# davidesantangelo/krep

Measured on AMD Instinct MI355X. Metric: GB/s scanned (literal scan, match offsets produced), haystack resident in HBM, higher is better.
Workload: dtype u8; 1 GPU; literal8: 8-byte case-sensitive literal 'Sherlock', ~1e-4 matches/byte, offsets tracked; 32 GiB per GPU (BASELINE.json configs[1]); pattern=Sherlock, bytes_per_gpu=34359738368, matches=3436005, parallelism=contiguous shards x1, start-offset ownership, 1 RCCL all-reduce of counts

## Files before the change

include/krep_gpu_debug.h:

```cpp
#ifndef KREP_GPU_DEBUG_H
#define KREP_GPU_DEBUG_H
#include "krep_gpu.h"
#ifdef __cplusplus
extern "C" {
#endif

uint64_t krep_gpu_debug_replay_host(int krep_ref_algo, const void *text, size_t n, const void *pattern, uint32_t m,
                                    int whole_word, size_t cur, int open_line);
void krep_gpu_debug_force_rounds(int rounds);
void krep_gpu_debug_force_stage_cap(int records);
void krep_gpu_debug_force_single_grid(int blocks);
uint64_t krep_gpu_debug_single_failovers(void);
uint64_t krep_gpu_debug_single_launches(void);
uint64_t krep_gpu_debug_tiny_launches(void);
uint64_t krep_gpu_debug_tiny_dense_launches(void);
void krep_gpu_debug_inject_failure(int kind);
void krep_gpu_debug_chain_fixups(uint64_t *rescans, uint64_t *replays);
void krep_gpu_debug_fold_carry(const krep_gpu_seq_carry_t *in, const krep_gpu_seq_carry_t *piece, krep_gpu_seq_carry_t *out);
uint64_t krep_gpu_debug_anchored_launches(void);
uint64_t krep_gpu_debug_literal_dma_launches(void);
int krep_gpu_debug_literal_dma_state(const krep_gpu_plan_t *plan, int *looked, int *barred, double *pass_rate);
uint64_t krep_gpu_debug_runs_launches(void);
int krep_gpu_debug_split_state(const krep_gpu_plan_t *plan);
int krep_gpu_debug_anchor_info(const krep_gpu_plan_t *plan, int *state, uint32_t *moved, double *rate_end_grams, double *rate_anchors);
int krep_gpu_debug_anchor_measured(const krep_gpu_plan_t *plan, double *measured, int *resamples);

#ifdef __cplusplus
}
#endif
#endif
```

krep_amd/csrc/kg_ac.hip:

```cpp
#include <hip/hip_runtime.h>

#include <algorithm>
#include <atomic>
#include <cstdlib>
#include <cstring>
#include <unordered_map>
#include <vector>

#include "../../include/krep_gpu.h"
#include "kg_ac_common.h"
#include "kg_ac_tables.h"
#include "kg_internal.h"

namespace kg {

#ifndef KG_AC_LINES_ROLL_CELLS
#define KG_AC_LINES_ROLL_CELLS 4
#endif
template <bool CI, bool LINES, bool SHORT, int STRIDE, int ANCH = 0, bool WW = false>
__global__ __launch_bounds__(kAcBlock) void ac_scan_kernel(const AcArgs a)
{
    static_assert(!WW || (STRIDE == 2 && !SHORT), "the -w filter of the depth masks: pair filter, no short patterns");
    static_assert(!ANCH || (STRIDE == 2 && !LINES && !SHORT), "anchored scan: pair filter, records / counts only");
    extern __shared__ __attribute__((aligned(16))) u32 s_mem[];
// ... 1177 lines not shown
    const u32 waves = r.tiny ? (u32)kTinyWaves : (u32)kAcWaves;
    a.upt = (u32)std::min<u64>(kAcUnitsPerTicketMax, std::max<u64>(1, a.num_tiles / ((u64)c.num_cu * waves * 4)));
    if (const char *e = getenv("KREP_GPU_AC_UPT"))
    {
        const int v = atoi(e);
        if (v >= 1 && v <= (int)kAcUnitsPerTicketMax)
            a.upt = (u32)v;
    }
    if (c.time_it) HIPCHK(hipEventRecord(c.ev0, c.st));
    const bool dbg_sync = getenv("KREP_GPU_SYNC_DEBUG") != nullptr;
    auto dbg = [&](const char *what) -> int {
        if (!dbg_sync)
            return 0;
        const hipError_t e = hipStreamSynchronize(c.st);
        return e == hipSuccess ? 0 : fail("ac_scan: %s faulted: %s (tiny=%d stride=%u units=%llu stage_cap=%u lines=%d list=%d own=[%llu,%llu) end=[%llu,%llu) n=%llu)", what,
                                          hipGetErrorString(e), (int)r.tiny, a.stride, (unsigned long long)n_units, a.stage_cap, (int)c.lines, (int)r.lines_on_list,
                                          (unsigned long long)a.own_lo, (unsigned long long)a.own_hi, (unsigned long long)a.end_lo,
                                          (unsigned long long)a.end_hi, (unsigned long long)c.text_len);
    };
    HIPCHK(hipMemsetAsync(c.d_ctr, 0, sizeof(Counters), c.st));
    HIPCHK(ac_staged_launch(c, r, a));
    if (dbg("scan kernel")) return 2;
    if (chain && post_order(*c.post, n_units, a.stage_cap, 0, a.anchor + c.global_base, kAcUnitBytes, c.lines, (uint64_t *)c.d_pos, r.want, c.d_ctr,
                            c.num_cu, c.st))
        return 2;
    if (dbg("post-pass")) return 2;
    if (r.lines_on_list && r.want && tail_launch_line_gaps(c.d_text, c.text_len, c.global_base, (const uint64_t *)c.d_pos, &c.d_ctr->total,
                                                           &c.d_ctr->overflow_units, r.want, &c.d_ctr->lines, c.st))
        return 2;
    if (dbg("line-gap kernel")) return 2;
    if (c.time_it) HIPCHK(hipEventRecord(c.ev1, c.st));
    HIPCHK(hipMemcpyAsync(c.h_ctr, c.d_ctr, sizeof(Counters), hipMemcpyDeviceToHost, c.st));
    HIPCHK(hipStreamSynchronize(c.st));
    return 0;
}
static void ac_learn(const AcScan &c, const AcRun &r)
{
    AcTables *t = c.t;
    const AcArgs &a = r.a;
    const Counters &h = *c.h_ctr;
    const size_t own_lo = c.own_lo, own_hi = r.own_hi;
    const u64 n_units = a.num_tiles;
    if (!r.tiny && !c.lines && a.stride == 2 && own_hi > own_lo)
    {
        const double tested = 0.5 * (double)(own_hi - own_lo);
        t->anch_measured = (double)h.candidates / tested;
        const double est = t->anch_state == 2 ? t->anch_rate : t->anch_rate0;
        if (t->anch_state != 0 && t->anch_resamples < kAnchResamples && c.text_len >= (1u << 20) && own_hi - own_lo >= (1u << 19) &&
            t->anch_measured > 0.008 && t->anch_measured > 2.0 * est + 0.002 && !getenv("KREP_GPU_AC_ANCHOR") && !getenv("KREP_GPU_AC_NO_RESAMPLE"))
        {
            if (getenv("KREP_GPU_DEBUG"))
                fprintf(stderr, "krep-gpu: anchors: measured %.3f %% candidates per tested position against %.3f %% estimated (%s): the next scan decides again\n",
                        100.0 * t->anch_measured, 100.0 * est, t->anch_state == 2 ? "anchored" : "end grams");
            t->anch_state = 0;
            ++t->anch_resamples;
        }
    }
    if (!r.want || r.fsc)
        return;
    if (r.tiny && h.overflow_units * 2 > n_units && h.total > n_units * 256)
        t->stage_cap = 0;
    else if (t->stage_cap && h.overflow_units * 64 > n_units)
        t->stage_cap = 64;
    else if (!t->stage_cap && h.total < n_units * 32)
        t->stage_cap = 64;
    if (r.tiny)
// ... 47 lines not shown
```

krep_amd/csrc/kg_internal.h:

```cpp
#pragma once
#include <hip/hip_runtime.h>

#include <atomic>
#include <cstring>
#include <initializer_list>
#include <mutex>
#include <vector>

#include "../../include/krep_gpu.h"
#include "../../include/krep_gpu_debug.h"
#include "kg_common.h"

namespace kg {

int fail(const char *fmt, ...);
const char *device_unusable(int device);
bool inject(int kind);
#define HIPCHK(x)                                                                                 \
    do                                                                                            \
    {                                                                                             \
        hipError_t e_ = (x);                                                                      \
        if (e_ != hipSuccess)                                                                     \
            return kg::fail("%s failed: %s (%s:%d)", #x, hipGetErrorString(e_), __FILE__, __LINE__); \
    } while (0)
// ... 29 lines not shown
    (void)hipGetDevice(&dev);
    const bool known = dev >= 0 && dev < 64;
    if (known && granted[dev].load(std::memory_order_acquire))
        return hipSuccess;
    const hipError_t e = hipFuncSetAttribute(reinterpret_cast<const void *>(Kernel), hipFuncAttributeMaxDynamicSharedMemorySize, bytes);
    if (e == hipSuccess && known)
        granted[dev].store(true, std::memory_order_release);
    return e;
}

hipError_t launch_literal(const LitArgs &a, uint32_t num_cu, hipStream_t st);
int runs_count_greedy(const uint8_t *d_text, uint64_t text_len, uint64_t lo, uint64_t hi, uint32_t m, uint8_t byte, bool ci, int num_cu,
                      unsigned long long *d_slots, unsigned long long *h_slots, hipStream_t st, uint64_t *total, uint64_t *end_p1);
bool literal_dma_eligible(const LitArgs &a);
hipError_t launch_literal_dma(const LitArgs &a, uint32_t num_cu, hipStream_t st);
hipError_t launch_dma_byte_look(const uint8_t *text, uint64_t lo, uint32_t n_cells, uint32_t prefilter, bool ci, unsigned long long *out, hipStream_t st);
extern std::atomic<uint64_t> g_runs_launches;
extern std::atomic<uint64_t> g_lit_dma_launches;

struct PostScratch;
constexpr int kFusedShapeMax = 5;
double single_fused_max_density(int shape);
int single_fused_shape_for(double density, double margin, int start);
bool single_fused_reopens(uint64_t total, uint64_t span);
constexpr int kFusedGaveUp = 1;
int single_fused_run(const LitArgs &a, uint64_t n_units, uint64_t span, PostScratch &post, Counters *d_ctr, Counters *h_ctr,
                     uint32_t num_cu, int *shape, hipEvent_t ev_end, hipStream_t st, bool count_launch);

struct PostScratch
{
    unsigned long long *d_unitinfo = nullptr;
    unsigned long long *d_offsets = nullptr;
    unsigned long long *d_blk = nullptr;
    uint64_t units_cap = 0;
    unsigned long long *d_stage = nullptr;
    uint64_t stage_cap_words = 0;
    uint64_t *d_occ = nullptr;
    uint64_t occ_cap = 0;
    uint8_t *d_keep = nullptr;
    unsigned long long *d_gblk = nullptr;
    unsigned long long *d_surv = nullptr;
    uint64_t keep_cap = 0;
    unsigned long long *d_tk = nullptr;
    uint64_t tk_cap = 0;
};
void post_free(PostScratch &s);
int post_reserve(PostScratch &s, uint64_t n_units, uint64_t stage_words);
int post_order(PostScratch &s, uint64_t n_units, uint32_t stage_cap, uint32_t fixed_len, uint64_t origin, uint64_t unit_bytes,
               bool want_lines, uint64_t *d_pos, uint64_t pos_cap, Counters *d_ctr, int num_cu, hipStream_t st);
int post_offsets_pass(PostScratch &s, uint64_t n_units, bool want_lines, Counters *d_ctr, hipStream_t st);
int post_gather_pass(PostScratch &s, uint64_t n_units, uint32_t stage_cap, uint32_t fixed_len, uint64_t origin,
                     uint64_t unit_bytes, uint64_t *d_pos, uint64_t pos_cap, int num_cu, hipStream_t st);
constexpr uint32_t kWalkGreedy = 0;
constexpr uint32_t kWalkShortO = 1;
constexpr uint32_t kWalkShortOLines = 2;
struct WalkSpec
{
    uint32_t mode, m;
    bool ww, lines, ci;
    uint8_t b1, b2;
};
int post_walk(PostScratch &s, const uint8_t *d_text, uint64_t text_len, uint64_t global_base, const WalkSpec &ws,
              uint64_t n_occ, uint64_t *d_pos, uint64_t want, Counters *d_ctr, Counters *h_ctr, hipStream_t st,
              uint64_t *total, uint64_t *nlines, uint64_t *resume);

constexpr uint32_t kNlWalkSse42 = 0, kNlWalkKmp = 1;
int post_nlwalk(PostScratch &s, const uint8_t *d_text, uint64_t text_len, uint32_t mode, uint32_t m, uint32_t k0, bool ww, bool om,
                uint64_t maxc, uint64_t n_occ, const uint64_t *d_lineno, Counters *d_ctr, Counters *h_ctr, hipStream_t st,
                uint64_t *count, uint64_t global_base, uint64_t global_len, uint64_t line_off, uint64_t cp_in, uint64_t seen_in,
                uint64_t *cp_out, uint64_t *seen_out);

struct ReplayIn;
int tail_last_hit(const unsigned long long *d_unitinfo, uint64_t limit_units, unsigned long long *d_slot,
                  unsigned long long *h_slot, hipStream_t st, uint64_t *unit_plus1);
int tail_find_next_newline(const uint8_t *d_text, uint64_t from, uint64_t n, unsigned long long *d_slot,
                           unsigned long long *h_slot, hipStream_t st, uint64_t *pos);
int tail_find_prev_newline(const uint8_t *d_text, uint64_t before, unsigned long long *d_slot, unsigned long long *h_slot,
                           hipStream_t st, uint64_t *pos_plus1);
int tail_count_changes(const uint64_t *d_v, uint64_t n, unsigned long long *d_slot, unsigned long long *h_slot, hipStream_t st,
                       uint64_t *changes);
int tail_count_line_gaps(const uint8_t *d_text, uint64_t text_len, uint64_t global_base, const uint64_t *d_rec, uint64_t n, unsigned long long *d_slot,
                         unsigned long long *h_slot, hipStream_t st, uint64_t *lines);
// ... 78 lines not shown
```

krep_amd/csrc/kg_post.hip:

```cpp
#include <hip/hip_runtime.h>
#include <cstdio>
#include <cstdlib>
#include <algorithm>
#include "kg_common.h"
#include "kg_device.h"
#include "kg_internal.h"

namespace kg {

constexpr int kPostBlock = 256;
constexpr int kPostUnitsPerThread = 4;
constexpr int kPostUnitsPerBlock = kPostBlock * kPostUnitsPerThread;

struct Bits { bool nl, head, tail; };
__device__ __forceinline__ Bits bits_of(u64 w) { return Bits{(w & kLnNl) != 0, (w & kLnHead) != 0, (w & kLnTail) != 0}; }
__device__ __forceinline__ u64 word_of(Bits b) { return (b.nl ? kLnNl : 0) | (b.head ? kLnHead : 0) | (b.tail ? kLnTail : 0); }
__device__ __forceinline__ Bits compose(Bits a, Bits b)
{
    return Bits{a.nl || b.nl, a.nl ? a.head : (a.head || b.head), b.nl ? b.tail : (a.tail || b.tail)};
}

__device__ __forceinline__ Bits wave_compose(Bits mine)
{
    const u64 nlm = __ballot(mine.nl), hdm = __ballot(mine.head), tlm = __ballot(mine.tail);
// ... 142 lines not shown
    for (int k = 0; k < kPostUnitsPerThread; ++k)
    {
        if (u0 + k < n_units)
        {
            offsets[u0 + k] = off;
            off += w[k] & kUiCountMask;
            if (want_lines)
            {
                const Bits ub = bits_of(w[k]);
                lines += (w[k] >> kUiLineShift) & kUiLineMask;
                if (lane_open && ub.head)
                    lines -= 1;
                lane_open = ub.nl ? ub.tail : (lane_open || ub.head);
            }
        }
    }
    if (want_lines)
    {
#pragma unroll
        for (int o = 32; o >= 1; o >>= 1)
            lines += __shfl_xor(lines, o);
        if (lane == 0)
            s_lines[wave] = lines;
        __syncthreads();
        if (threadIdx.x == 0)
        {
            const u64 t = s_lines[0] + s_lines[1] + s_lines[2] + s_lines[3];
            if (t)
                atomicAdd(&ctr->lines, t);
        }
    }
}

__global__ __launch_bounds__(kPostBlock) void post_gather(const u64 *__restrict__ info, u64 n_units,
                                                          const u64 *__restrict__ offsets, const u64 *__restrict__ stage,
                                                          u32 stage_cap, u32 fixed_len, u64 origin, u64 unit_bytes,
                                                          u64 *__restrict__ positions, u64 pos_cap)
{
    const unsigned short *stage16 = reinterpret_cast<const unsigned short *>(stage);
    const u32 lane = lane_id();
    const u64 n_waves = (u64)gridDim.x * (kPostBlock / 64);
    const u64 wid = (u64)blockIdx.x * (kPostBlock / 64) + (threadIdx.x >> 6);
    const u32 *stage32 = reinterpret_cast<const u32 *>(stage);
    auto put = [&](u64 idx, u64 org, u64 sbase, u32 i) {
        u64 s, e;
        if (fixed_len)
        {
            s = org + stage16[sbase + i];
            e = s + fixed_len;
        }
        else
        {
            const u32 w = stage32[sbase + i];
            s = org + (u64)(w >> 11) - 1024ull;
            e = s + (w & 2047u);
        }
        *reinterpret_cast<uint4 *>(positions + 2 * idx) = make_uint4((u32)s, (u32)(s >> 32), (u32)e, (u32)(e >> 32));
    };
    for (u64 g = wid * 64; g < n_units; g += n_waves * 64)
    {
        const u64 u = g + lane;
        u32 cnt = 0;
        u64 off = 0;
        if (u < n_units)
        {
            cnt = (u32)(info[u] & kUiCountMask);
            off = offsets[u];
            if (cnt > stage_cap || off >= pos_cap)
                cnt = 0;
        }
        if (!fixed_len)
        {
            const u32 raw = u < n_units ? (u32)(info[u] & kUiCountMask) : 0u;
            u32 incl = raw;
#pragma unroll
            for (int o = 1; o < 64; o <<= 1)
            {
                const u32 t = __shfl_up(incl, o);
                if (lane >= (u32)o)
                    incl += t;
            }
            const u32 total = __shfl(incl, 63);
            const u64 off0 = __shfl(u < n_units ? offsets[u] : 0ull, 0);
            for (u32 j0 = 0; j0 < total; j0 += 64u)
            {
                const u32 j = j0 + lane;
                u32 own = 0;
#pragma unroll
                for (u32 step = 32; step; step >>= 1)
                {
                    const u32 t = __shfl(incl, (own + step - 1u) & 63u);
                    if (t <= j)
                        own += step;
                }
                own &= 63u;
                const u32 oincl = __shfl(incl, own), oraw = __shfl(raw, own);
                const u32 i = j - (oincl - oraw);
                const u64 idx = off0 + j;
                if (j < total && oraw <= stage_cap && idx < pos_cap)
                    put(idx, origin + (g + (u64)own) * unit_bytes, (g + (u64)own) * (u64)stage_cap, i);
            }
            continue;
        }
        if (cnt && cnt <= 4u)
        {
            const u64 sbase = u * (u64)stage_cap, org = origin + u * unit_bytes;
            for (u32 i = 0; i < cnt; ++i)
                if (off + i < pos_cap)
                    put(off + i, org, sbase, i);
            cnt = 0;
        }
        u64 big = __ballot(cnt != 0);
        if (fixed_len && stage_cap <= 512)
        {
            while (big)
            {
                const int l = __builtin_ctzll(big);
                big &= big - 1;
                const u32 c = __shfl(cnt, l);
                const u64 o = __shfl(off, l);
                const u64 sbase = (g + (u64)l) * (u64)stage_cap, org = origin + (g + (u64)l) * unit_bytes;
                u32 v[8];
#pragma unroll
                for (int k = 0; k < 8; ++k)
                {
                    const u32 i = lane + 64u * (u32)k;
                    v[k] = stage16[sbase + (i < c ? i : c - 1u)];
                }
#pragma unroll
                for (int k = 0; k < 8; ++k)
                {
                    const u32 i = lane + 64u * (u32)k;
                    if (i < c && o + i < pos_cap)
                    {
                        const u64 s0 = org + v[k], e0 = s0 + fixed_len;
                        *reinterpret_cast<uint4 *>(positions + 2 * (o + i)) = make_uint4((u32)s0, (u32)(s0 >> 32), (u32)e0, (u32)(e0 >> 32));
                    }
                }
            }
        }
        while (big)
        {
            const int l = __builtin_ctzll(big);
            big &= big - 1;
            const u32 c = __shfl(cnt, l);
            const u64 o = __shfl(off, l);
            const u64 sbase = (g + (u64)l) * (u64)stage_cap, org = origin + (g + (u64)l) * unit_bytes;
            for (u32 i = lane; i < c; i += 64)
                if (o + i < pos_cap)
                    put(o + i, org, sbase, i);
        }
    }
}

void post_free(PostScratch &s)
{
    if (s.d_unitinfo) (void)hipFree(s.d_unitinfo);
    if (s.d_offsets) (void)hipFree(s.d_offsets);
    if (s.d_blk) (void)hipFree(s.d_blk);
    if (s.d_stage) (void)hipFree(s.d_stage);
    if (s.d_occ) (void)hipFree(s.d_occ);
    if (s.d_keep) (void)hipFree(s.d_keep);
    if (s.d_gblk) (void)hipFree(s.d_gblk);
    if (s.d_surv) (void)hipFree(s.d_surv);
    if (s.d_tk) (void)hipFree(s.d_tk);
    s = PostScratch{};
}

int post_reserve(PostScratch &s, uint64_t n_units, uint64_t stage_words)
{
    const uint64_t nb = (n_units + kPostUnitsPerBlock - 1) / kPostUnitsPerBlock;
    HIPCHK(grow_scratch(s.units_cap, n_units, n_units,
                        {dev_buf(s.d_unitinfo, n_units * sizeof(u64)), dev_buf(s.d_offsets, n_units * sizeof(u64)), dev_buf(s.d_blk, 2 * nb * sizeof(u64))}));
    HIPCHK(grow_scratch(s.stage_cap_words, stage_words, stage_words, {dev_buf(s.d_stage, stage_words * sizeof(u64))}));
    if (getenv("KREP_GPU_DEBUG_ALLOC"))
        fprintf(stderr, "[krep_gpu] scratch: unitinfo %p offsets %p blk %p stage %p (%llu units, %llu stage words)\n", (void *)s.d_unitinfo,
                (void *)s.d_offsets, (void *)s.d_blk, (void *)s.d_stage, (unsigned long long)s.units_cap, (unsigned long long)s.stage_cap_words);
    return 0;
}

int post_offsets_pass(PostScratch &s, uint64_t n_units, bool want_lines, Counters *d_ctr, hipStream_t st)
{
    const uint64_t nb = (n_units + kPostUnitsPerBlock - 1) / kPostUnitsPerBlock;
    u64 *blk_sum = (u64 *)s.d_blk, *blk_bits = (u64 *)s.d_blk + nb;
    hipLaunchKernelGGL(post_reduce, dim3((u32)nb), dim3(kPostBlock), 0, st, (const u64 *)s.d_unitinfo, (u64)n_units, blk_sum,
                       blk_bits);
    hipLaunchKernelGGL(post_carry, dim3(1), dim3(64), 0, st, (u64)nb, blk_sum, blk_bits, d_ctr);
    hipLaunchKernelGGL(post_offsets, dim3((u32)nb), dim3(kPostBlock), 0, st, (const u64 *)s.d_unitinfo, (u64)n_units,
                       (const u64 *)blk_sum, (const u64 *)blk_bits, (u64 *)s.d_offsets, d_ctr, want_lines ? 1 : 0);
    HIPCHK(hipGetLastError());
    return 0;
}

int post_gather_pass(PostScratch &s, uint64_t n_units, uint32_t stage_cap, uint32_t fixed_len, uint64_t origin,
                     uint64_t unit_bytes, uint64_t *d_pos, uint64_t pos_cap, int num_cu, hipStream_t st)
{
    if (!d_pos || !pos_cap)
        return 0;
    const uint64_t groups = (n_units + 63) / 64;
    const u32 grid = (u32)std::min<uint64_t>((groups + 3) / 4, (uint64_t)num_cu * 16);
    hipLaunchKernelGGL(post_gather, dim3(grid ? grid : 1), dim3(kPostBlock), 0, st, (const u64 *)s.d_unitinfo, (u64)n_units,
                       (const u64 *)s.d_offsets, (const u64 *)s.d_stage, stage_cap, fixed_len, (u64)origin, (u64)unit_bytes,
                       (u64 *)d_pos, (u64)pos_cap);
    HIPCHK(hipGetLastError());
    return 0;
}

int post_order(PostScratch &s, uint64_t n_units, uint32_t stage_cap, uint32_t fixed_len, uint64_t origin, uint64_t unit_bytes,
               bool want_lines, uint64_t *d_pos, uint64_t pos_cap, Counters *d_ctr, int num_cu, hipStream_t st)
{
    if (post_offsets_pass(s, n_units, want_lines, d_ctr, st))
        return 2;
    if (stage_cap == 0 && pos_cap)
        return 0;
    return post_gather_pass(s, n_units, stage_cap, fixed_len, origin, unit_bytes, d_pos, pos_cap, num_cu, st);
}

}
```

krep_amd/csrc/kg_scan.hip:

```cpp
#include <hip/hip_runtime.h>

#include <algorithm>
#include <cstdio>
#include <cstdlib>
#include <cstring>
#include <vector>

#include "../../include/krep_gpu.h"
#include "kg_common.h"
#include "kg_internal.h"
#include "kg_plan.h"
#include "kg_replay.h"

using namespace kg;

struct Verdict { uint64_t ret, store; };
static Verdict verdict_for(int algo, const krep_gpu_plan *pl, uint64_t total, uint64_t lines, bool have_result)
{
    const size_t maxc = pl->max_count;
    const bool store = pl->track && have_result;
    Verdict v{0, 0};
    switch (algo)
    {
    case KREP_RA_MEMCHR:
// ... 307 lines not shown
        const double density = L.density(pl->h_ctr->total);
        if (density * 32768.0 >= fusedk_min_hits_per_unit() && density <= single_fused_max_density(kFusedShapeMax))
        {
            pl->fusedk_on = true;
            pl->fusedk_shape = single_fused_shape_for(density, 1.0, 0);
        }
    }
    if (getenv("KREP_GPU_DEBUG") && (a.flags & F_POS))
        fprintf(stderr, "krep-gpu: literal scan: %llu of %llu units overflowed a %u-entry slot (fullest: %llu); one-pass next: %d (shape %d)\n",
                pl->h_ctr->overflow_units, (unsigned long long)L.n_units, a.stage_cap, pl->h_ctr->max_unit_count, (int)pl->fusedk_on,
                pl->fusedk_shape);
}
static void lit_reopen(krep_gpu_plan *pl, const LitScan &L)
{
    const uint32_t m_scan = L.a.m;
    if (!pl->fused1_ok && m_scan == 1 && single_fused_reopens(pl->h_ctr->total, L.span()))
        pl->fused1_ok = true;
    if (pl->fusedk_never && m_scan >= 2 && m_scan <= 8 && single_fused_reopens(pl->h_ctr->total, L.span()))
        pl->fusedk_never = false;
}

static int lit_two_pass(krep_gpu_plan *pl, const Window &w, const LitPass &ps, LitScan &L, bool chain, hipStream_t st)
{
    LitArgs &a = L.a;
    a.positions = ps.d_out;
    a.pos_cap = ps.sink == LitPass::RECORDS ? ps.out_cap : 0;
    HIPCHK(launch_literal(a, (uint32_t)pl->num_cu, st));
    if (chain && post_order(*ps.post, L.n_units, a.stage_cap, a.m, a.anchor + w.global_base, L.unit_bytes(), ps.lines, ps.d_out, a.pos_cap,
                            pl->d_ctr, pl->num_cu, st))
        return 2;
    if (ps.ev_end) HIPCHK(hipEventRecord(ps.ev_end, st));
    HIPCHK(hipMemcpyAsync(pl->h_ctr, pl->d_ctr, sizeof(Counters), hipMemcpyDeviceToHost, st));
    HIPCHK(hipStreamSynchronize(st));
    lit_dma_rate(pl, w, L);
    lit_learn_density(pl, ps, L);
    if ((a.flags & F_POS) && pl->h_ctr->overflow_units)
    {
        LitArgs e = a;
        e.emit_mode = 1;
        HIPCHK(hipMemsetAsync(&pl->d_ctr->ticket, 0, sizeof(unsigned long long), st));
        HIPCHK(launch_literal(e, (uint32_t)pl->num_cu, st));
        if (ps.ev_end) HIPCHK(hipEventRecord(ps.ev_end, st));
    }
    return 0;
}
static int lit_two_pass_occ(krep_gpu_plan *pl, const Window &w, const LitPass &ps, const LitScan &L, hipStream_t st)
{
    const LitArgs &a = L.a;
    PostScratch &post = *ps.post;
    HIPCHK(launch_literal(a, (uint32_t)pl->num_cu, st));
    if (post_offsets_pass(post, L.n_units, false, pl->d_ctr, st))
        return 2;
    HIPCHK(hipMemcpyAsync(pl->h_ctr, pl->d_ctr, sizeof(Counters), hipMemcpyDeviceToHost, st));
    HIPCHK(hipStreamSynchronize(st));
    const uint64_t n_occ = pl->h_ctr->total;
    HIPCHK(grow_scratch(post.occ_cap, n_occ, n_occ, {dev_buf(post.d_occ, n_occ * 2 * sizeof(uint64_t))}));
    if (n_occ)
    {
        if (post_gather_pass(post, L.n_units, a.stage_cap, a.m, a.anchor + w.global_base, L.unit_bytes(), post.d_occ, n_occ, pl->num_cu, st))
            return 2;
        if (pl->h_ctr->overflow_units)
        {
            LitArgs e = a;
            e.emit_mode = 1;
            e.positions = post.d_occ;
            e.pos_cap = n_occ;
// ... 822 lines not shown
```

krep_amd/engine.py:

```python
from __future__ import annotations

import ctypes as C
import os

import numpy as np

from . import abi

HERE = os.path.dirname(os.path.abspath(__file__))
LIB_PATH = os.path.join(HERE, "lib", "libkrep_gpu.so")


class KrepGpuError(RuntimeError):
    pass


class Engine:

    def __init__(self, path: str = LIB_PATH):
        path = os.environ.get("KREP_GPU_LIB", path)
        if not os.path.exists(path):
            raise KrepGpuError(f"{path} is missing: build it with `python -m krep_amd.build` "
                               "(hipcc --offload-arch=gfx950); there is no CPU fallback")
        if not os.environ.get("KREP_GPU_NO_TORCH"):
# ... 84 lines not shown
        L.krep_gpu_comm_allreduce_u64.argtypes = [C.POINTER(C.c_uint64), C.c_int]
        L.krep_gpu_comm_allreduce_device_u64.restype = C.c_int
        L.krep_gpu_comm_allreduce_device_u64.argtypes = [C.c_void_p, C.c_int, C.c_void_p]
        L.krep_gpu_comm_destroy.restype = None
        L.krep_gpu_rccl_calls.restype = C.c_uint64
        L.krep_gpu_rccl_version.restype = C.c_int
        L.krep_gpu_debug_force_single_grid.restype = None
        L.krep_gpu_debug_force_single_grid.argtypes = [C.c_int]
        L.krep_gpu_debug_single_failovers.restype = C.c_uint64
        L.krep_gpu_debug_single_launches.restype = C.c_uint64
        L.krep_gpu_debug_tiny_launches.restype = C.c_uint64
        L.krep_gpu_debug_chain_fixups.restype = None
        L.krep_gpu_debug_chain_fixups.argtypes = [C.POINTER(C.c_uint64), C.POINTER(C.c_uint64)]
        L.krep_gpu_debug_tiny_dense_launches.restype = C.c_uint64
        if hasattr(L, "krep_gpu_debug_anchor_info"):
            L.krep_gpu_debug_anchored_launches.restype = C.c_uint64
            L.krep_gpu_debug_literal_dma_launches.restype = C.c_uint64
            L.krep_gpu_debug_runs_launches.restype = C.c_uint64
            L.krep_gpu_debug_anchor_info.restype = C.c_int
            L.krep_gpu_debug_anchor_info.argtypes = [C.c_void_p, C.POINTER(C.c_int), C.POINTER(C.c_uint32), C.POINTER(C.c_double),
                                                     C.POINTER(C.c_double)]
        if hasattr(L, "krep_gpu_alloc_placed"):
            L.krep_gpu_alloc_placed.restype = C.c_int
            L.krep_gpu_alloc_placed.argtypes = [C.c_int, C.c_size_t, C.c_size_t, C.c_int, C.POINTER(C.c_void_p), C.POINTER(C.c_void_p),
                                                C.POINTER(abi.Placement)]
            L.krep_gpu_free_placed.restype = C.c_int
            L.krep_gpu_free_placed.argtypes = [C.c_int, C.c_void_p]
        if hasattr(L, "krep_gpu_debug_literal_dma_state"):
            L.krep_gpu_debug_literal_dma_state.restype = C.c_int
            L.krep_gpu_debug_literal_dma_state.argtypes = [C.c_void_p, C.POINTER(C.c_int), C.POINTER(C.c_int), C.POINTER(C.c_double)]
        if hasattr(L, "krep_gpu_debug_anchor_measured"):
            L.krep_gpu_debug_anchor_measured.restype = C.c_int
            L.krep_gpu_debug_anchor_measured.argtypes = [C.c_void_p, C.POINTER(C.c_double), C.POINTER(C.c_int)]
        L.krep_gpu_last_shard_info.restype = None
        L.krep_gpu_last_shard_info.argtypes = [C.POINTER(abi.ShardInfo)]
        L.krep_gpu_available.restype = C.c_int
        L.krep_gpu_unavailable_reason.restype = C.c_char_p
        L.krep_gpu_last_status.restype = C.c_int
        L.krep_gpu_set_cpu_fallback.restype = None
        L.krep_gpu_set_cpu_fallback.argtypes = [C.c_void_p]
        L.krep_gpu_worthwhile.restype = C.c_int
        L.krep_gpu_worthwhile.argtypes = [C.POINTER(abi.SearchParams), C.c_size_t]
        L.krep_gpu_worthwhile_ex.restype = C.c_int
        L.krep_gpu_worthwhile_ex.argtypes = [C.POINTER(abi.SearchParams), C.c_size_t, C.c_int]
        L.krep_gpu_cost_estimate.restype = C.c_int
        L.krep_gpu_cost_estimate.argtypes = [C.POINTER(abi.SearchParams), C.c_size_t, C.c_int, C.POINTER(abi.Cost)]
        L.krep_gpu_get_cost_rates.restype = None
        L.krep_gpu_get_cost_rates.argtypes = [C.POINTER(abi.CostRates)]
        L.krep_gpu_set_cost_rates.restype = None
        L.krep_gpu_set_cost_rates.argtypes = [C.POINTER(abi.CostRates)]
        L.krep_gpu_set_min_text_bytes.restype = None
        L.krep_gpu_set_min_text_bytes.argtypes = [C.c_size_t]
        L.krep_gpu_device_count.restype = C.c_int
        L.krep_gpu_last_error.restype = C.c_char_p
        L.krep_gpu_clear_error.restype = None
        L.krep_gpu_version.restype = C.c_char_p

    def set_reference_simd(self, level: int):
        self.lib.krep_gpu_set_reference_simd(level)

    def set_only_matching(self, on: bool):
        self.lib.krep_gpu_set_only_matching(int(on))

    def set_force_no_simd(self, on: bool):
        self.lib.krep_gpu_set_force_no_simd(int(on))

# ... 63 lines not shown
        return self.lib.krep_gpu_select_search_algorithm(params.ref)

    def available(self) -> bool:
        return bool(self.lib.krep_gpu_available())

    def unavailable_reason(self) -> str:
        return (self.lib.krep_gpu_unavailable_reason() or b"").decode()

    def last_status(self) -> int:
        return int(self.lib.krep_gpu_last_status())

    def set_cpu_fallback(self, selector_address):
        self.lib.krep_gpu_set_cpu_fallback(C.c_void_p(selector_address) if selector_address else None)

    def worthwhile(self, params: abi.Params, text_len: int) -> bool:
        return bool(self.lib.krep_gpu_worthwhile(params.ref, text_len))

    def worthwhile_ex(self, params: abi.Params, text_len: int, cpu_threads: int) -> bool:
        return bool(self.lib.krep_gpu_worthwhile_ex(params.ref, text_len, cpu_threads))

    def cost_estimate(self, params: abi.Params, text_len: int, cpu_threads: int = 0) -> "abi.Cost":
        c = abi.Cost()
        if self.lib.krep_gpu_cost_estimate(params.ref, text_len, cpu_threads, C.byref(c)):
            raise KrepGpuError("krep_gpu_cost_estimate failed")
        return c

    def cost_rates(self) -> "abi.CostRates":
        r = abi.CostRates()
        self.lib.krep_gpu_get_cost_rates(C.byref(r))
        return r

    def set_cost_rates(self, rates: "abi.CostRates | None"):
        self.lib.krep_gpu_set_cost_rates(C.byref(rates) if rates is not None else None)

    def inject_failure(self, kind: int):
        self.lib.krep_gpu_debug_inject_failure(kind)

    def set_num_gpus(self, n: int):
        self.lib.krep_gpu_set_num_gpus(n)

    def comm_unique_id(self) -> bytes:
        buf = C.create_string_buffer(128)
        if self.lib.krep_gpu_comm_unique_id(buf):
            raise KrepGpuError("krep_gpu_comm_unique_id failed: " + self.last_error())
        return buf.raw

    def comm_init_rank(self, id128: bytes, nranks: int, rank: int, device: int):
        assert len(id128) == 128
        buf = C.create_string_buffer(id128, 128)
        if self.lib.krep_gpu_comm_init_rank(buf, nranks, rank, device):
            raise KrepGpuError("krep_gpu_comm_init_rank failed: " + self.last_error())

    def comm_allreduce(self, values):
        arr = (C.c_uint64 * len(values))(*[int(v) for v in values])
        if self.lib.krep_gpu_comm_allreduce_u64(arr, len(values)):
            raise KrepGpuError("krep_gpu_comm_allreduce_u64 failed: " + self.last_error())
        return [int(v) for v in arr]

    def comm_destroy(self):
        self.lib.krep_gpu_comm_destroy()

    def rccl_calls(self) -> int:
        return int(self.lib.krep_gpu_rccl_calls())

    def rccl_version(self) -> int:
        return int(self.lib.krep_gpu_rccl_version())
# ... 223 lines not shown
```

Before: 6575 GB/s.

## Replace multi-pass post ordering with single-pass decoupled look-back scan and fused gather

```diff
diff --git a/include/krep_gpu_debug.h b/include/krep_gpu_debug.h
--- a/include/krep_gpu_debug.h
+++ b/include/krep_gpu_debug.h
@@ -15,6 +15,7 @@
 uint64_t krep_gpu_debug_tiny_launches(void);
 uint64_t krep_gpu_debug_tiny_dense_launches(void);
 void krep_gpu_debug_inject_failure(int kind);
+uint64_t krep_gpu_debug_post_failovers(void);
 void krep_gpu_debug_chain_fixups(uint64_t *rescans, uint64_t *replays);
 void krep_gpu_debug_fold_carry(const krep_gpu_seq_carry_t *in, const krep_gpu_seq_carry_t *piece, krep_gpu_seq_carry_t *out);
 uint64_t krep_gpu_debug_anchored_launches(void);
diff --git a/krep_amd/csrc/kg_ac.hip b/krep_amd/csrc/kg_ac.hip
--- a/krep_amd/csrc/kg_ac.hip
+++ b/krep_amd/csrc/kg_ac.hip
@@ -1233,6 +1233,18 @@
     if (c.time_it) HIPCHK(hipEventRecord(c.ev1, c.st));
     HIPCHK(hipMemcpyAsync(c.h_ctr, c.d_ctr, sizeof(Counters), hipMemcpyDeviceToHost, c.st));
     HIPCHK(hipStreamSynchronize(c.st));
+    if (chain && post_gave_up(c.h_ctr))
+    {
+        if (post_redo_chain(*c.post, n_units, a.stage_cap, 0, a.anchor + c.global_base, kAcUnitBytes, c.lines, (uint64_t *)c.d_pos, r.want, c.d_ctr,
+                            c.num_cu, c.st))
+            return 2;
+        if (r.lines_on_list && r.want && tail_launch_line_gaps(c.d_text, c.text_len, c.global_base, (const uint64_t *)c.d_pos, &c.d_ctr->total,
+                                                               &c.d_ctr->overflow_units, r.want, &c.d_ctr->lines, c.st))
+            return 2;
+        if (c.time_it) HIPCHK(hipEventRecord(c.ev1, c.st));
+        HIPCHK(hipMemcpyAsync(c.h_ctr, c.d_ctr, sizeof(Counters), hipMemcpyDeviceToHost, c.st));
+        HIPCHK(hipStreamSynchronize(c.st));
+    }
     return 0;
 }
 static void ac_learn(const AcScan &c, const AcRun &r)
diff --git a/krep_amd/csrc/kg_internal.h b/krep_amd/csrc/kg_internal.h
--- a/krep_amd/csrc/kg_internal.h
+++ b/krep_amd/csrc/kg_internal.h
@@ -85,6 +85,9 @@
     unsigned long long *d_unitinfo = nullptr;
     unsigned long long *d_offsets = nullptr;
     unsigned long long *d_blk = nullptr;
+    unsigned long long *d_look = nullptr;
+    uint64_t look_epoch = 0;
+    uint64_t look_drawn = 0;
     uint64_t units_cap = 0;
     unsigned long long *d_stage = nullptr;
     uint64_t stage_cap_words = 0;
@@ -101,6 +104,11 @@
 int post_reserve(PostScratch &s, uint64_t n_units, uint64_t stage_words);
 int post_order(PostScratch &s, uint64_t n_units, uint32_t stage_cap, uint32_t fixed_len, uint64_t origin, uint64_t unit_bytes,
                bool want_lines, uint64_t *d_pos, uint64_t pos_cap, Counters *d_ctr, int num_cu, hipStream_t st);
+constexpr unsigned long long kPostGaveUp = 1ull;
+bool post_gave_up(const Counters *h_ctr);
+int post_redo_chain(PostScratch &s, uint64_t n_units, uint32_t stage_cap, uint32_t fixed_len, uint64_t origin, uint64_t unit_bytes,
+                    bool want_lines, uint64_t *d_pos, uint64_t pos_cap, Counters *d_ctr, int num_cu, hipStream_t st);
+extern std::atomic<uint64_t> g_post_failovers;
 int post_offsets_pass(PostScratch &s, uint64_t n_units, bool want_lines, Counters *d_ctr, hipStream_t st);
 int post_gather_pass(PostScratch &s, uint64_t n_units, uint32_t stage_cap, uint32_t fixed_len, uint64_t origin,
                      uint64_t unit_bytes, uint64_t *d_pos, uint64_t pos_cap, int num_cu, hipStream_t st);
diff --git a/krep_amd/csrc/kg_post.hip b/krep_amd/csrc/kg_post.hip
--- a/krep_amd/csrc/kg_post.hip
+++ b/krep_amd/csrc/kg_post.hip
@@ -198,16 +198,21 @@
     }
 }
 
-__global__ __launch_bounds__(kPostBlock) void post_gather(const u64 *__restrict__ info, u64 n_units,
-                                                          const u64 *__restrict__ offsets, const u64 *__restrict__ stage,
-                                                          u32 stage_cap, u32 fixed_len, u64 origin, u64 unit_bytes,
-                                                          u64 *__restrict__ positions, u64 pos_cap)
-{
-    const unsigned short *stage16 = reinterpret_cast<const unsigned short *>(stage);
-    const u32 lane = lane_id();
-    const u64 n_waves = (u64)gridDim.x * (kPostBlock / 64);
-    const u64 wid = (u64)blockIdx.x * (kPostBlock / 64) + (threadIdx.x >> 6);
-    const u32 *stage32 = reinterpret_cast<const u32 *>(stage);
+struct Gather
+{
+    const u64 *stage;
+    u32 stage_cap, fixed_len;
+    u64 origin, unit_bytes;
+    u64 *positions;
+    u64 pos_cap, n_units;
+};
+__device__ __forceinline__ void gather_group(const Gather &ga, const u64 g, const u32 lane, const u32 raw, const u64 off)
+{
+    const unsigned short *stage16 = reinterpret_cast<const unsigned short *>(ga.stage);
+    const u32 *stage32 = reinterpret_cast<const u32 *>(ga.stage);
+    const u32 stage_cap = ga.stage_cap, fixed_len = ga.fixed_len;
+    const u64 origin = ga.origin, unit_bytes = ga.unit_bytes, pos_cap = ga.pos_cap;
+    u64 *const positions = ga.positions;
     auto put = [&](u64 idx, u64 org, u64 sbase, u32 i) {
         u64 s, e;
         if (fixed_len)
@@ -223,88 +228,66 @@
         }
         *reinterpret_cast<uint4 *>(positions + 2 * idx) = make_uint4((u32)s, (u32)(s >> 32), (u32)e, (u32)(e >> 32));
     };
-    for (u64 g = wid * 64; g < n_units; g += n_waves * 64)
-    {
-        const u64 u = g + lane;
-        u32 cnt = 0;
-        u64 off = 0;
-        if (u < n_units)
-        {
-            cnt = (u32)(info[u] & kUiCountMask);
-            off = offsets[u];
-            if (cnt > stage_cap || off >= pos_cap)
-                cnt = 0;
-        }
-        if (!fixed_len)
-        {
-            const u32 raw = u < n_units ? (u32)(info[u] & kUiCountMask) : 0u;
-            u32 incl = raw;
-#pragma unroll
-            for (int o = 1; o < 64; o <<= 1)
+    const u64 u = g + lane;
+    u32 cnt = raw;
+    if (cnt > stage_cap || off >= pos_cap)
+        cnt = 0;
+    if (!fixed_len)
+    {
+        u32 incl = raw;
+#pragma unroll
+        for (int o = 1; o < 64; o <<= 1)
+        {
+            const u32 t = __shfl_up(incl, o);
+            if (lane >= (u32)o)
+                incl += t;
+        }
+        const u32 total = __shfl(incl, 63);
+        const u64 off0 = __shfl(off, 0);
+        for (u32 j0 = 0; j0 < total; j0 += 64u)
+        {
+            const u32 j = j0 + lane;
+            u32 own = 0;
+#pragma unroll
+            for (u32 step = 32; step; step >>= 1)
             {
-                const u32 t = __shfl_up(incl, o);
-                if (lane >= (u32)o)
-                    incl += t;
+                const u32 t = __shfl(incl, (own + step - 1u) & 63u);
+                if (t <= j)
+                    own += step;
             }
-            const u32 total = __shfl(incl, 63);
-            const u64 off0 = __shfl(u < n_units ? offsets[u] : 0ull, 0);
-            for (u32 j0 = 0; j0 < total; j0 += 64u)
-            {
-                const u32 j = j0 + lane;
-                u32 own = 0;
-#pragma unroll
-                for (u32 step = 32; step; step >>= 1)
+            own &= 63u;
+            const u32 oincl = __shfl(incl, own), oraw = __shfl(raw, own);
+            const u32 i = j - (oincl - oraw);
+            const u64 idx = off0 + j;
+            if (j < total && oraw <= stage_cap && idx < pos_cap)
+                put(idx, origin + (g + (u64)own) * unit_bytes, (g + (u64)own) * (u64)stage_cap, i);
+        }
+        return;
+    }
+    if (cnt && cnt <= 4u)
+    {
+        const u64 sbase = u * (u64)stage_cap, org = origin + u * unit_bytes;
+        if (fixed_len && !(stage_cap & 3u))
+        {
+            const uint2 q = *reinterpret_cast<const uint2 *>(stage16 + sbase);
+            const u32 rel[4] = {q.x & 0xffffu, q.x >> 16, q.y & 0xffffu, q.y >> 16};
+#pragma unroll
+            for (u32 i = 0; i < 4u; ++i)
+                if (i < cnt && off + i < pos_cap)
                 {
-                    const u32 t = __shfl(incl, (own + step - 1u) & 63u);
-                    if (t <= j)
-                        own += step;
+                    const u64 s0 = org + rel[i], e0 = s0 + fixed_len;
+                    *reinterpret_cast<uint4 *>(positions + 2 * (off + i)) = make_uint4((u32)s0, (u32)(s0 >> 32), (u32)e0, (u32)(e0 >> 32));
                 }
-                own &= 63u;
-                const u32 oincl = __shfl(incl, own), oraw = __shfl(raw, own);
-                const u32 i = j - (oincl - oraw);
-                const u64 idx = off0 + j;
-                if (j < total && oraw <= stage_cap && idx < pos_cap)
-                    put(idx, origin + (g + (u64)own) * unit_bytes, (g + (u64)own) * (u64)stage_cap, i);
-            }
-            continue;
-        }
-        if (cnt && cnt <= 4u)
-        {
-            const u64 sbase = u * (u64)stage_cap, org = origin + u * unit_bytes;
+        }
+        else
             for (u32 i = 0; i < cnt; ++i)
                 if (off + i < pos_cap)
                     put(off + i, org, sbase, i);
-            cnt = 0;
-        }
-        u64 big = __ballot(cnt != 0);
-        if (fixed_len && stage_cap <= 512)
-        {
-            while (big)
-            {
-                const int l = __builtin_ctzll(big);
-                big &= big - 1;
-                const u32 c = __shfl(cnt, l);
-                const u64 o = __shfl(off, l);
-                const u64 sbase = (g + (u64)l) * (u64)stage_cap, org = origin + (g + (u64)l) * unit_bytes;
-                u32 v[8];
-#pragma unroll
-                for (int k = 0; k < 8; ++k)
-                {
-                    const u32 i = lane + 64u * (u32)k;
-                    v[k] = stage16[sbase + (i < c ? i : c - 1u)];
-                }
-#pragma unroll
-                for (int k = 0; k < 8; ++k)
-                {
-                    const u32 i = lane + 64u * (u32)k;
-                    if (i < c && o + i < pos_cap)
-                    {
-                        const u64 s0 = org + v[k], e0 = s0 + fixed_len;
-                        *reinterpret_cast<uint4 *>(positions + 2 * (o + i)) = make_uint4((u32)s0, (u32)(s0 >> 32), (u32)e0, (u32)(e0 >> 32));
-                    }
-                }
-            }
-        }
+        cnt = 0;
+    }
+    u64 big = __ballot(cnt != 0);
+    if (fixed_len && stage_cap <= 512)
+    {
         while (big)
         {
             const int l = __builtin_ctzll(big);
@@ -312,18 +295,257 @@
             const u32 c = __shfl(cnt, l);
             const u64 o = __shfl(off, l);
             const u64 sbase = (g + (u64)l) * (u64)stage_cap, org = origin + (g + (u64)l) * unit_bytes;
-            for (u32 i = lane; i < c; i += 64)
-                if (o + i < pos_cap)
-                    put(o + i, org, sbase, i);
-        }
-    }
-}
+            u32 v[8];
+#pragma unroll
+            for (int k = 0; k < 8; ++k)
+            {
+                const u32 i = lane + 64u * (u32)k;
+                v[k] = stage16[sbase + (i < c ? i : c - 1u)];
+            }
+#pragma unroll
+            for (int k = 0; k < 8; ++k)
+            {
+                const u32 i = lane + 64u * (u32)k;
+                if (i < c && o + i < pos_cap)
+                {
+                    const u64 s0 = org + v[k], e0 = s0 + fixed_len;
+                    *reinterpret_cast<uint4 *>(positions + 2 * (o + i)) = make_uint4((u32)s0, (u32)(s0 >> 32), (u32)e0, (u32)(e0 >> 32));
+                }
+            }
+        }
+    }
+    while (big)
+    {
+        const int l = __builtin_ctzll(big);
+        big &= big - 1;
+        const u32 c = __shfl(cnt, l);
+        const u64 o = __shfl(off, l);
+        const u64 sbase = (g + (u64)l) * (u64)stage_cap, org = origin + (g + (u64)l) * unit_bytes;
+        for (u32 i = lane; i < c; i += 64)
+            if (o + i < pos_cap)
+                put(o + i, org, sbase, i);
+    }
+}
+
+__global__ __launch_bounds__(kPostBlock) void post_gather(const u64 *__restrict__ info, const u64 *__restrict__ offsets, const Gather ga)
+{
+    const u32 lane = lane_id();
+    const u64 n_waves = (u64)gridDim.x * (kPostBlock / 64);
+    const u64 wid = (u64)blockIdx.x * (kPostBlock / 64) + (threadIdx.x >> 6);
+    for (u64 g = wid * 64; g < ga.n_units; g += n_waves * 64)
+    {
+        const u64 u = g + lane;
+        const bool live = u < ga.n_units;
+        gather_group(ga, g, lane, live ? (u32)(info[u] & kUiCountMask) : 0u, live ? offsets[u] : 0ull);
+    }
+}
+
+constexpr u64 kLbAgg = 1ull << 62, kLbIncl = 2ull << 62;
+constexpr int kLbEpochShift = 40, kLbEpochBits = 19;
+constexpr u64 kLbHitMask = (1ull << kLbEpochShift) - 1, kLbEpochMask = ((1ull << kLbEpochBits) - 1) << kLbEpochShift;
+constexpr u32 kLbSpinLimit = 1u << 22;
+constexpr u32 kLbMinUnitsPerBlock = 256;
+constexpr u32 kLbStateAt = 16;
+
+struct Prefix { u64 sum; Bits b; };
+__device__ __forceinline__ u64 lb_word(u64 state, u64 tag, Prefix p) { return state | tag | (word_of(p.b) >> 2) | (p.sum & kLbHitMask); }
+
+constexpr int kLbLook = 4;
+__device__ __forceinline__ Prefix lb_look_back(const u64 *state, const u64 blk, const u64 tag, const u32 spin_limit, Counters *ctr,
+                                               const u32 lane)
+{
+    Prefix acc{0, Bits{false, false, false}};
+    long long hi = (long long)blk - 1;
+    u32 spins = 0;
+    while (hi >= 0)
+    {
+        if (spins >= spin_limit)
+        {
+            if (lane == 0)
+                atomicOr(&ctr->summary, kPostGaveUp);
+            return Prefix{0, Bits{false, false, false}};
+        }
+        u64 w[kLbLook];
+#pragma unroll
+        for (int r = 0; r < kLbLook; ++r)
+        {
+            const long long mine = hi - 63 - 64 * r + (long long)lane;
+            w[r] = kLbIncl | tag;
+            if (mine >= 0)
+                w[r] = __hip_atomic_load(&state[mine], __ATOMIC_RELAXED, __HIP_MEMORY_SCOPE_AGENT);
+        }
+        bool met = false, missing = false;
+#pragma unroll
+        for (int r = 0; r < kLbLook; ++r)
+        {
+            if (met || missing)
+                break;
+            const bool fresh = (w[r] & kLbEpochMask) == tag && (w[r] >> 62) != 0;
+            const u64 incl_m = __ballot(fresh && (w[r] >> 62) == 2), stale_m = __ballot(!fresh);
+            const u32 first = incl_m ? 63u - (u32)__builtin_clzll(incl_m) : 0u;
+            if (stale_m >> first)
+            {
+                missing = true;
+                break;
+            }
+            const bool take = lane >= first;
+            u64 s = take ? (w[r] & kLbHitMask) : 0ull;
+#pragma unroll
+            for (int o = 32; o >= 1; o >>= 1)
+                s += __shfl_xor(s, o);
+            const Bits wb = wave_compose(take ? bits_of(w[r] << 2) : Bits{false, false, false});
+            acc.sum += s;
+            acc.b = compose(wb, acc.b);
+            met = incl_m != 0;
+            hi -= 64;
+        }
+        if (met)
+            break;
+        if (missing)
+        {
+            ++spins;
+            __builtin_amdgcn_s_sleep(2);
+        }
+    }
+    return acc;
+}
+
+template <int T, int K>
+__global__ __launch_bounds__(T) void post_one(const u64 *__restrict__ info, const u64 n_units, u64 *look, const u64 drawn_before,
+                                              const u64 tag, const u32 spin_limit, u64 *__restrict__ offsets, Counters *ctr,
+                                              const int want_lines, const int gather, const Gather ga)
+{
+    constexpr int W = T / 64, G = W * K;
+    static_assert(G <= 64 && T * K >= (int)kLbMinUnitsPerBlock, "one wave scans the groups; the state words are sized for 256-unit blocks");
+    __shared__ u64 s_blk;
+    __shared__ u64 s_goff[G];
+    __shared__ u64 s_gbits[G];
+    __shared__ u64 s_lines[W];
+    const u32 lane = lane_id(), wave = threadIdx.x >> 6;
+    if (threadIdx.x == 0)
+        s_blk = __hip_atomic_fetch_add(&look[0], 1ull, __ATOMIC_RELAXED, __HIP_MEMORY_SCOPE_AGENT) - drawn_before;
+    __syncthreads();
+    const u64 blk = s_blk, n_blocks = gridDim.x;
+    if (blk >= n_blocks)
+    {
+        if (threadIdx.x == 0)
+            atomicOr(&ctr->summary, kPostGaveUp);
+        return;
+    }
+    u64 *state = look + kLbStateAt;
+    const u64 ub = blk * (u64)(T * K);
+    u64 w[K];
+    u32 incl[K];
+#pragma unroll
+    for (int k = 0; k < K; ++k)
+    {
+        const u64 u = ub + (u64)(k * T) + threadIdx.x;
+        w[k] = u < n_units ? info[u] : 0ull;
+    }
+#pragma unroll
+    for (int k = 0; k < K; ++k)
+    {
+        u32 c = (u32)(w[k] & kUiCountMask);
+#pragma unroll
+        for (int o = 1; o < 64; o <<= 1)
+        {
+            const u32 v = __shfl_up(c, o);
+            if (lane >= (u32)o)
+                c += v;
+        }
+        incl[k] = c;
+        const Bits gb = wave_compose(bits_of(w[k]));
+        if (lane == 63)
+            s_goff[k * W + wave] = c;
+        if (lane == 0)
+            s_gbits[k * W + wave] = word_of(gb);
+    }
+    __syncthreads();
+    if (wave == 0)
+    {
+        const bool live = lane < (u32)G;
+        const u64 gs = live ? s_goff[lane] : 0ull;
+        const Bits gb = live ? bits_of(s_gbits[lane]) : Bits{false, false, false};
+        u64 gi = gs;
+#pragma unroll
+        for (int o = 1; o < 64; o <<= 1)
+        {
+            const u64 v = __shfl_up(gi, o);
+            if (lane >= (u32)o)
+                gi += v;
+        }
+        const Prefix agg{__shfl(gi, 63), wave_compose(gb)};
+        if (blk && lane == 0)
+            __hip_atomic_store(&state[blk], lb_word(kLbAgg, tag, agg), __ATOMIC_RELAXED, __HIP_MEMORY_SCOPE_AGENT);
+        const Prefix ex = lb_look_back(state, blk, tag, spin_limit, ctr, lane);
+        const Prefix in{ex.sum + agg.sum, compose(ex.b, agg.b)};
+        if (lane == 0)
+        {
+            __hip_atomic_store(&state[blk], lb_word(kLbIncl, tag, in), __ATOMIC_RELAXED, __HIP_MEMORY_SCOPE_AGENT);
+            if (blk + 1 == n_blocks)
+                atomicOr(&ctr->summary, word_of(in.b));
+        }
+        const bool open = wave_open_in(gb, ex.b.tail, lane);
+        if (live)
+        {
+            s_goff[lane] = ex.sum + (gi - gs);
+            s_gbits[lane] = open ? 1ull : 0ull;
+        }
+    }
+    __syncthreads();
+    u64 off[K];
+    u64 lines = 0;
+#pragma unroll
+    for (int k = 0; k < K; ++k)
+    {
+        const u64 u = ub + (u64)(k * T) + threadIdx.x;
+        const Bits ub_ = bits_of(w[k]);
+        off[k] = s_goff[k * W + wave] + (u64)(incl[k] - (u32)(w[k] & kUiCountMask));
+        const bool lane_open = wave_open_in(ub_, s_gbits[k * W + wave] != 0, lane);
+        if (u < n_units)
+        {
+            offsets[u] = off[k];
+            lines += (w[k] >> kUiLineShift) & kUiLineMask;
+            if (lane_open && ub_.head)
+                lines -= 1;
+        }
+    }
+    if (want_lines)
+    {
+#pragma unroll
+        for (int o = 32; o >= 1; o >>= 1)
+            lines += __shfl_xor(lines, o);
+        if (lane == 0)
+            s_lines[wave] = lines;
+        __syncthreads();
+        if (threadIdx.x == 0)
+        {
+            u64 t = 0;
+            for (int q = 0; q < W; ++q)
+                t += s_lines[q];
+            if (t)
+                atomicAdd(&ctr->lines, t);
+        }
+    }
+    if (!gather)
+        return;
+#pragma unroll
+    for (int k = 0; k < K; ++k)
+    {
+        const u64 g = ub + (u64)(k * T) + (u64)wave * 64u;
+        if (g < n_units)
+            gather_group(ga, g, lane, (u32)(w[k] & kUiCountMask), off[k]);
+    }
+}
+
+static uint64_t post_look_words(uint64_t units) { return ((kLbStateAt + units / kLbMinUnitsPerBlock + 1) + 15) / 16 * 16; }
 
 void post_free(PostScratch &s)
 {
     if (s.d_unitinfo) (void)hipFree(s.d_unitinfo);
     if (s.d_offsets) (void)hipFree(s.d_offsets);
     if (s.d_blk) (void)hipFree(s.d_blk);
+    if (s.d_look) (void)hipFree(s.d_look);
     if (s.d_stage) (void)hipFree(s.d_stage);
     if (s.d_occ) (void)hipFree(s.d_occ);
     if (s.d_keep) (void)hipFree(s.d_keep);
@@ -335,9 +557,12 @@
 
 int post_reserve(PostScratch &s, uint64_t n_units, uint64_t stage_words)
 {
-    const uint64_t nb = (n_units + kPostUnitsPerBlock - 1) / kPostUnitsPerBlock;
+    const uint64_t nb = (n_units + kPostUnitsPerBlock - 1) / kPostUnitsPerBlock, cap_before = s.units_cap;
     HIPCHK(grow_scratch(s.units_cap, n_units, n_units,
-                        {dev_buf(s.d_unitinfo, n_units * sizeof(u64)), dev_buf(s.d_offsets, n_units * sizeof(u64)), dev_buf(s.d_blk, 2 * nb * sizeof(u64))}));
+                        {dev_buf(s.d_unitinfo, n_units * sizeof(u64)), dev_buf(s.d_offsets, n_units * sizeof(u64)), dev_buf(s.d_blk, 2 * nb * sizeof(u64)),
+                         dev_buf(s.d_look, post_look_words(n_units) * sizeof(u64))}));
+    if (s.units_cap != cap_before)
+        s.look_epoch = 0;
     HIPCHK(grow_scratch(s.stage_cap_words, stage_words, stage_words, {dev_buf(s.d_stage, stage_words * sizeof(u64))}));
     if (getenv("KREP_GPU_DEBUG_ALLOC"))
         fprintf(stderr, "[krep_gpu] scratch: unitinfo %p offsets %p blk %p stage %p (%llu units, %llu stage words)\n", (void *)s.d_unitinfo,
@@ -365,15 +590,14 @@
         return 0;
     const uint64_t groups = (n_units + 63) / 64;
     const u32 grid = (u32)std::min<uint64_t>((groups + 3) / 4, (uint64_t)num_cu * 16);
-    hipLaunchKernelGGL(post_gather, dim3(grid ? grid : 1), dim3(kPostBlock), 0, st, (const u64 *)s.d_unitinfo, (u64)n_units,
-                       (const u64 *)s.d_offsets, (const u64 *)s.d_stage, stage_cap, fixed_len, (u64)origin, (u64)unit_bytes,
-                       (u64 *)d_pos, (u64)pos_cap);
+    const Gather ga{(const u64 *)s.d_stage, stage_cap, fixed_len, (u64)origin, (u64)unit_bytes, (u64 *)d_pos, (u64)pos_cap, (u64)n_units};
+    hipLaunchKernelGGL(post_gather, dim3(grid ? grid : 1), dim3(kPostBlock), 0, st, (const u64 *)s.d_unitinfo, (const u64 *)s.d_offsets, ga);
     HIPCHK(hipGetLastError());
     return 0;
 }
 
-int post_order(PostScratch &s, uint64_t n_units, uint32_t stage_cap, uint32_t fixed_len, uint64_t origin, uint64_t unit_bytes,
-               bool want_lines, uint64_t *d_pos, uint64_t pos_cap, Counters *d_ctr, int num_cu, hipStream_t st)
+static int post_order_chain(PostScratch &s, uint64_t n_units, uint32_t stage_cap, uint32_t fixed_len, uint64_t origin, uint64_t unit_bytes,
+                            bool want_lines, uint64_t *d_pos, uint64_t pos_cap, Counters *d_ctr, int num_cu, hipStream_t st)
 {
     if (post_offsets_pass(s, n_units, want_lines, d_ctr, st))
         return 2;
@@ -382,4 +606,64 @@
     return post_gather_pass(s, n_units, stage_cap, fixed_len, origin, unit_bytes, d_pos, pos_cap, num_cu, st);
 }
 
-}
+std::atomic<uint64_t> g_post_failovers{0};
+
+template <int T, int K>
+static void launch_post_one(PostScratch &s, uint64_t n_units, u32 spin_limit, bool want_lines, bool gather, const Gather &ga, Counters *d_ctr,
+                            hipStream_t st)
+{
+    const uint64_t nb = (n_units + (uint64_t)(T * K) - 1) / (uint64_t)(T * K);
+    hipLaunchKernelGGL((post_one<T, K>), dim3((u32)nb), dim3(T), 0, st, (const u64 *)s.d_unitinfo, (u64)n_units, (u64 *)s.d_look,
+                       (u64)s.look_drawn, (u64)s.look_epoch << kLbEpochShift, spin_limit, (u64 *)s.d_offsets, d_ctr, want_lines ? 1 : 0,
+                       gather ? 1 : 0, ga);
+    s.look_drawn += nb;
+}
+
+int post_order(PostScratch &s, uint64_t n_units, uint32_t stage_cap, uint32_t fixed_len, uint64_t origin, uint64_t unit_bytes,
+               bool want_lines, uint64_t *d_pos, uint64_t pos_cap, Counters *d_ctr, int num_cu, hipStream_t st)
+{
+    const char *e = getenv("KREP_GPU_POST_CHAIN");
+    if ((e && atoi(e)) || !n_units)
+        return post_order_chain(s, n_units, stage_cap, fixed_len, origin, unit_bytes, want_lines, d_pos, pos_cap, d_ctr, num_cu, st);
+    if (s.look_epoch == 0 || s.look_epoch + 1 >= (1ull << kLbEpochBits))
+    {
+        HIPCHK(hipMemsetAsync(s.d_look, 0, post_look_words(s.units_cap) * sizeof(u64), st));
+        s.look_epoch = 0;
+        s.look_drawn = 0;
+    }
+    ++s.look_epoch;
+    const bool gather = d_pos && pos_cap && !(stage_cap == 0 && pos_cap);
+    const Gather ga{(const u64 *)s.d_stage, stage_cap, fixed_len, (u64)origin, (u64)unit_bytes, (u64 *)d_pos, (u64)pos_cap, (u64)n_units};
+    const u32 spin_limit = inject(5) ? 0u : kLbSpinLimit;
+    int shape = 0;
+    if (const char *sh = getenv("KREP_GPU_POST_SHAPE"))
+        shape = atoi(sh);
+    switch (shape)
+    {
+    case 2564: launch_post_one<256, 4>(s, n_units, spin_limit, want_lines, gather, ga, d_ctr, st); break;
+    case 2562: launch_post_one<256, 2>(s, n_units, spin_limit, want_lines, gather, ga, d_ctr, st); break;
+    case 2561: launch_post_one<256, 1>(s, n_units, spin_limit, want_lines, gather, ga, d_ctr, st); break;
+    case 5122: launch_post_one<512, 2>(s, n_units, spin_limit, want_lines, gather, ga, d_ctr, st); break;
+    case 5121: launch_post_one<512, 1>(s, n_units, spin_limit, want_lines, gather, ga, d_ctr, st); break;
+    case 10244: launch_post_one<1024, 4>(s, n_units, spin_limit, want_lines, gather, ga, d_ctr, st); break;
+    case 5124: launch_post_one<512, 4>(s, n_units, spin_limit, want_lines, gather, ga, d_ctr, st); break;
+    case 10241: launch_post_one<1024, 1>(s, n_units, spin_limit, want_lines, gather, ga, d_ctr, st); break;
+    case 10242: launch_post_one<1024, 2>(s, n_units, spin_limit, want_lines, gather, ga, d_ctr, st); break;
+    default: launch_post_one<1024, 2>(s, n_units, spin_limit, want_lines, gather, ga, d_ctr, st); break;
+    }
+    HIPCHK(hipGetLastError());
+    return 0;
+}
+
+bool post_gave_up(const Counters *h_ctr) { return (h_ctr->summary & kPostGaveUp) != 0; }
+
+int post_redo_chain(PostScratch &s, uint64_t n_units, uint32_t stage_cap, uint32_t fixed_len, uint64_t origin, uint64_t unit_bytes,
+                    bool want_lines, uint64_t *d_pos, uint64_t pos_cap, Counters *d_ctr, int num_cu, hipStream_t st)
+{
+    g_post_failovers.fetch_add(1);
+    HIPCHK(hipMemsetAsync(&d_ctr->lines, 0, sizeof(unsigned long long), st));
+    return post_order_chain(s, n_units, stage_cap, fixed_len, origin, unit_bytes, want_lines, d_pos, pos_cap, d_ctr, num_cu, st);
+}
+
+}
+extern "C" uint64_t krep_gpu_debug_post_failovers(void) { return kg::g_post_failovers.load(); }
diff --git a/krep_amd/csrc/kg_scan.hip b/krep_amd/csrc/kg_scan.hip
--- a/krep_amd/csrc/kg_scan.hip
+++ b/krep_amd/csrc/kg_scan.hip
@@ -363,6 +363,15 @@
     if (ps.ev_end) HIPCHK(hipEventRecord(ps.ev_end, st));
     HIPCHK(hipMemcpyAsync(pl->h_ctr, pl->d_ctr, sizeof(Counters), hipMemcpyDeviceToHost, st));
     HIPCHK(hipStreamSynchronize(st));
+    if (chain && post_gave_up(pl->h_ctr))
+    {
+        if (post_redo_chain(*ps.post, L.n_units, a.stage_cap, a.m, a.anchor + w.global_base, L.unit_bytes(), ps.lines, ps.d_out, a.pos_cap,
+                            pl->d_ctr, pl->num_cu, st))
+            return 2;
+        if (ps.ev_end) HIPCHK(hipEventRecord(ps.ev_end, st));
+        HIPCHK(hipMemcpyAsync(pl->h_ctr, pl->d_ctr, sizeof(Counters), hipMemcpyDeviceToHost, st));
+        HIPCHK(hipStreamSynchronize(st));
+    }
     lit_dma_rate(pl, w, L);
     lit_learn_density(pl, ps, L);
     if ((a.flags & F_POS) && pl->h_ctr->overflow_units)
diff --git a/krep_amd/engine.py b/krep_amd/engine.py
--- a/krep_amd/engine.py
+++ b/krep_amd/engine.py
@@ -140,6 +140,8 @@
         if hasattr(L, "krep_gpu_debug_anchor_measured"):
             L.krep_gpu_debug_anchor_measured.restype = C.c_int
             L.krep_gpu_debug_anchor_measured.argtypes = [C.c_void_p, C.POINTER(C.c_double), C.POINTER(C.c_int)]
+        if hasattr(L, "krep_gpu_debug_post_failovers"):
+            L.krep_gpu_debug_post_failovers.restype = C.c_uint64
         L.krep_gpu_last_shard_info.restype = None
         L.krep_gpu_last_shard_info.argtypes = [C.POINTER(abi.ShardInfo)]
         L.krep_gpu_available.restype = C.c_int
@@ -269,6 +271,9 @@
 
     def set_cost_rates(self, rates: "abi.CostRates | None"):
         self.lib.krep_gpu_set_cost_rates(C.byref(rates) if rates is not None else None)
+
+    def post_failovers(self) -> int:
+        return int(self.lib.krep_gpu_debug_post_failovers())
 
     def inject_failure(self, kind: int):
         self.lib.krep_gpu_debug_inject_failure(kind)
```

New measurement: 6612 GB/s, median of 6. About the same (+0.6%).
